# kemingy/rabitq

Hardware: AMD Instinct MI355X
Metric: queries/sec at recall@10>=0.95, 100Mx128; HBM GB/s on popcount scan (higher is better)
Workload: dtype exact integer dot (fp6 MFMA, v_dot8_u32_u4) + f32

## Files before the change

rabitq_amd/csrc/host_query.h:

```cpp
#pragma once
struct QueryParams {
    uint32_t nq, len, probe, topk;
    bool heuristic;
    uint32_t cap, hcap;
    const float *thr_init = nullptr;
    bool seg_final = false;
    bool ext_lists = false;
};

#define RQ_DEFAULT_CAP 4096u
#define RQ_MAX_CAP_HINT 32768u
#define RQ_MAX_NQ_PER_PASS 65536u
#define RQ_MAX_PROBE 16384u

static rq_status ws_prepare(const rq_index *idx, Workspace &ws, const QueryParams &qp) {
    const uint32_t nprobe = std::min(qp.probe, idx->k);
    const uint64_t nq = qp.nq, npairs = nq * nprobe;
    if (!ws.stream) HIPC(hipStreamCreateWithFlags(&ws.stream, hipStreamNonBlocking));
    if (!ws.h_totals) HIPC(hipHostMalloc((void **)&ws.h_totals, 16 * sizeof(unsigned long long)));
    RQC(ws.qpad.ensure(nq * idx->dim));
    RQC(ws.y.ensure(nq * idx->dim));
    if (!qp.ext_lists) RQC(ws.dist.ensure(nq * idx->k));
    RQC(ws.probe_dist.ensure(npairs));
    RQC(ws.probe_cluster.ensure(npairs));
// ... 418 lines not shown
        a.dbg = (uint32_t)g_scan_dbg.load();
        const uint32_t stage_tile = use_mfma ? scan_mfma_tile(W, arena_stage, additive) : tile;
        a.tiles_per_group = ceil_div(std::min<uint64_t>(idx->max_list_len, sg.s_hi), stage_tile);
        sp.tile_table = nullptr;
        const uint64_t grid_blocks = (uint64_t)k * a.tiles_per_group, real_tiles = idx->n / stage_tile + k;
        const int tt_opt = g_scan_tile_table.load();
        if (cluster_major && scan_is_fused(W) && sg.s_hi >= idx->max_list_len &&
            (tt_opt == 2 || (tt_opt == 1 && grid_blocks > 4 * real_tiles))) {
            uint32_t count = 0;
            sp.tile_table = get_tile_table(idx, stage_tile, &count);
            if (sp.tile_table) a.use_table = 1u, a.ngroups = count, a.tiles_per_group = 1u;
        }
        uint32_t dense_cells = 0;
        if (rq_large_batch(nq) && !use_mfma && scan_is_fused(W) && g_dense_dir.load() && sg.s_hi != 0xFFFFFFFFu &&
            !(qp.seg_final && span > qp.cap)) {
            const uint64_t cells = (uint64_t)((sg.s_hi - 1) >> 6) - (sg.s_lo >> 6) + 2ull * slot_hi + 2;
            if (cells <= qp.cap) dense_cells = (uint32_t)cells;
        }
        a.dense_dir = dense_cells ? 1u : 0u;
        QSeg seg = useg;
        bool runs_in_tmp = false;
        if (arena_stage) {
            uint64_t want = std::max<uint64_t>(idx->arena_hint.load(), (uint64_t)nq * qp.cap / 2);
            unsigned long long total_slots = 0;
            uint32_t arena_rsub = 0;
            bool arena_retried = false;
            ws.arena_failed = true;
#ifdef RQ_DEV_ABLATIONS
            if (g_seg_opt.load() == 3) {
                DevBuf<SurvRec> never;
                RQC(never.alloc(1ull << 46));
                return fail(RQ_ERR_OOM, "survivor arena: injected failure (developer hook survivor_segments = 3)");
            }
#endif
            for (int attempt = 0;; ++attempt) {
                want = std::min<uint64_t>(want, 0xFFFF0000ull);
                RQC(ws.arena_recs.ensure(want));
                RQC(ws.arena_runs.ensure(want));
                RQC(ws.arena_cur.ensure(RQ_ARENA_SHARDS + 4));
                RQC(ws.arena_fail.ensure(RQ_ARENA_SHARDS));
                HIPC(hipMemsetAsync(ws.arena_cur.p, 0, (RQ_ARENA_SHARDS + 4) * 8, st));
                HIPC(hipMemsetAsync(ws.arena_fail.p, 0xFF, RQ_ARENA_SHARDS * 4, st));
                ScanExtra hx{};
                RQC(ws.arena_places.ensure(want));
                hx.arena_places = ws.arena_places.p, hx.reserved = nullptr;
                hx.arena_recs = ws.arena_recs.p, hx.arena_runs = reinterpret_cast<uint4 *>(ws.arena_runs.p), hx.arena_cur = ws.arena_cur.p;
                hx.arena_fail = ws.arena_fail.p;
                {
                    const uint64_t have = std::min<uint64_t>(ws.arena_recs.count, ws.arena_runs.count);
                    hx.arena_sub = hx.arena_rsub = (uint32_t)(have * 7 / 8 / RQ_ARENA_SHARDS);
                    hx.arena_common = (uint32_t)std::min<uint64_t>(have - (uint64_t)hx.arena_sub * RQ_ARENA_SHARDS, 0xFFFFFF00ull);
                }
                arena_rsub = hx.arena_rsub;
                RQC(ws.scan_extra.ensure(1));
                HIPC(hipMemcpyAsync(ws.scan_extra.p, &hx, sizeof hx, hipMemcpyHostToDevice, st));
                a.x = ws.scan_extra.p;
                a.dense_dir = 0u;
                pf.begin(use_mfma ? PF_SCAN_MATRIX : PF_SCAN);
                if (use_mfma) launch_scan_mfma(sp, a, W, st, additive);
                else launch_scan(sp, a, W, st);
                pf.end();
                pf.begin(PF_GROUP);
                seg_exact_kernel<<<ceil_div(nq, 256), 256, 0, st>>>(ws.surv_cnt.p, nq, 64u, ws.q_cap.p);
                seg_scan_kernel<<<1, 1024, 0, st>>>(ws.q_cap.p, nq, ws.q_base.p, ws.arena_cur.p + RQ_ARENA_SHARDS + 1);
                unsigned long long tail[2] = {0, 0};
                HIPC(hipMemcpyAsync(tail, ws.arena_cur.p + RQ_ARENA_SHARDS, 16, hipMemcpyDeviceToHost, st));
                HIPC(hipStreamSynchronize(st));
                total_slots = tail[1];
                if (!(uint32_t)tail[0]) break;
                pf.end();
                if (attempt >= 6 || want >= 0xFFFF0000ull) return fail(RQ_ERR_OOM, "survivor arena kept overflowing");
                const uint64_t nblocks = a.use_table ? a.ngroups : (uint64_t)a.ngroups * a.tiles_per_group;
                HIPC(hipMemsetAsync(ws.surv_cnt.p, 0, (size_t)nq * sizeof(unsigned long long), st));
                want = std::max<uint64_t>(want * 2, 1u << 20);
                if (nblocks < RQ_ARENA_SHARDS) want = std::max<uint64_t>(want, 8 * total_slots + (1u << 16)), arena_retried = true;
                else want = std::max<uint64_t>(want, total_slots + total_slots / 4);
            }
            ws.arena_failed = false;
            {
                uint64_t cur = idx->arena_hint.load();
                const uint64_t learnt = std::max<uint64_t>(total_slots + total_slots * 3 / 5, arena_retried ? std::min<uint64_t>(want, 0xFFFF0000ull) : 0ull);
                while (cur < learnt && !const_cast<rq_index *>(idx)->arena_hint.compare_exchange_weak(cur, learnt)) {}
            }
            if (total_slots > ws.surv.count || total_slots > ws.runs.count || total_slots > ws.runs_tmp.count) {
                const uint64_t grow = total_slots + total_slots / 8;
                RQC(ws.surv.ensure(grow));
                RQC(ws.runs.ensure(grow));
                RQC(ws.runs_tmp.ensure(grow));
            }
            sp.surv = ws.surv.p, sp.runs = ws.runs.p;
            arena_scatter_kernel<<<dim3(RQ_ARENA_SHARDS + RQ_ARENA_COMMON_BLOCKS, 2), 256, 0, st>>>(ws.arena_recs.p, reinterpret_cast<const uint4 *>(ws.arena_runs.p), ws.arena_cur.p,
                                                                              ws.arena_fail.p, arena_rsub, ws.q_base.p, ws.arena_places.p, ws.surv.p, ws.runs_tmp.p);
            runs_in_tmp = true;
            pf.end();
            seg = QSeg{ws.q_base.p, ws.q_cap.p, qp.cap};
            ws.pend_seg_slots = std::max<uint64_t>(ws.pend_seg_slots, total_slots);
        }
        if (dense_cells) {
            pf.begin(PF_SORT);
            clear_dir_kernel<<<ceil_div((uint64_t)nq * dense_cells, 256), 256, 0, st>>>(ws.runs.p, nq, seg, dense_cells);
            pf.end();
        }
        if (!arena_stage) {
            pf.begin(use_mfma ? PF_SCAN_MATRIX : PF_SCAN);
            if (use_mfma) launch_scan_mfma(sp, a, W, st, additive);
            else launch_scan(sp, a, W, st);
            pf.end();
        }
        if (use_mfma) ws.pend_matrix_stages++;
        if (prof_acc && additive) prof_acc->matrix_additive_launches++;
        if (prof_acc) prof_acc->scan_launches++;
        if (prof_acc && use_mfma) {
            prof_acc->matrix_launches++;
            ws.pend_matrix_ranges.push_back({sg.s_lo, sg.s_hi});
        }
        if (!rq_large_batch(nq) && qp.cap <= 4 * RQ_DEFAULT_CAP) {
            pf.begin(PF_RERANK);
            const uint32_t fin_threads = nq <= 16 ? 1024u : 256u;
            const uint32_t presorted = qp.cap > RQ_DEFAULT_CAP && nprobe <= 1024 ? 1u : 0u;
            if (presorted) {
                sort_runs_kernel<<<nq, 64, 0, st>>>(ws.runs.p, ws.surv_cnt.p, seg, ws.big_list.p, ws.big_list.p + nq, RQ_SORT_LDS_RECS, nullptr);
                sort_runs_mid_kernel<<<std::min(nq, 256u), 256, RQ_SORT_MID_LDS_WORDS * 8, st>>>(ws.runs.p, ws.use_runs_tmp ? ws.runs_tmp.p : nullptr, ws.surv_cnt.p,
                                                                                              seg, ws.big_list.p, ws.big_list.p + nq, nprobe, 0u,
                                                                                              RQ_SORT_MID_LDS_WORDS);
            }
            if (sb_fused_finish) {
                uint32_t flags = presorted;
                if (nq <= 32) {
                    accurate_kernel<<<dim3(std::max(1u, std::min(16u, 256u / nq)), nq), 256, (size_t)dim * sizeof(float), st>>>(
                        ws.surv.p, ws.surv_cnt.p, seg, idx->view(), qpad, dim, nullptr, probe_cluster, nprobe);
                    flags |= 2u;
                }
                const uint32_t presorted = flags;
                if (topk < 64)
                    sb_finish_kernel<true><<<nq, fin_threads, (size_t)dim * sizeof(float) + (2 * RQ_SBF_RUNS + RQ_SBF_RECS) * 16, st>>>(
                        ws.surv.p, ws.runs.p, ws.surv_cnt.p, seg, idx->view(), qpad, dim, topk, rs, probe_cluster, nprobe, presorted,
                        idx->map_ids.p, d_out_dist, d_out_id, d_out_n, ws.rough_cnt.p, ws.totals.p);
                else
                    sb_finish_kernel<false><<<nq, fin_threads, (size_t)dim * sizeof(float) + (2 * RQ_SBF_RUNS + RQ_SBF_RECS) * 16, st>>>(
                        ws.surv.p, ws.runs.p, ws.surv_cnt.p, seg, idx->view(), qpad, dim, topk, rs, probe_cluster, nprobe, presorted,
                        idx->map_ids.p, d_out_dist, d_out_id, d_out_n, ws.rough_cnt.p, ws.totals.p);
                sb_results_done = true;
            } else if (qp.heuristic)
                stage_finish_kernel<true><<<nq, fin_threads, (size_t)dim * sizeof(float), st>>>(ws.surv.p, ws.runs.p, ws.surv_cnt.p, seg, idx->view(),
                                                              qpad, dim, topk, rs, probe_cluster, nprobe, presorted);
            else
                stage_finish_kernel<false><<<nq, fin_threads, (size_t)dim * sizeof(float), st>>>(ws.surv.p, ws.runs.p, ws.surv_cnt.p, seg, idx->view(),
                                                               qpad, dim, topk, rs, probe_cluster, nprobe, presorted);
            pf.end();
        } else {
            pf.begin(PF_RERANK);
            const uint32_t gx = std::max(1u, std::min(16u, 4096u / std::max(nq, 1u)));
            if (idx->base_q8.p && (stage_no > 0 || qp.thr_init) && !(g_scan_dbg & 512))
                accurate_filtered8_kernel<<<dim3(gx, nq), 256, (size_t)dim * sizeof(float) + (nprobe <= RQ_ACC8_LDS_PROBES ? (size_t)nprobe * 16 : 0), st>>>(
                    ws.surv.p, ws.surv_cnt.p, seg, idx->base.p, idx->base_q8.p, idx->list_q8.p, qpad, dim, rerank_order, ws.thr.p,
                    probe_cluster, nprobe, ws.nshadow.p, k);
            else if (idx->base_h.p && (stage_no > 0 || qp.thr_init) && !(g_scan_dbg & 512))
                accurate_filtered_kernel<<<dim3(gx, nq), 256, (size_t)dim * sizeof(float), st>>>(
                    ws.surv.p, ws.surv_cnt.p, seg, idx->base.p, idx->base_h.p, qpad, dim, rerank_order, ws.thr.p,
                    ws.nshadow.p);
            else if (idx->split_rows && (stage_no > 0 || qp.thr_init) && !(g_scan_dbg & 512))
                accurate_split_kernel<<<dim3(gx, nq), 256, (size_t)dim * sizeof(float) + (nprobe <= RQ_ACC8_LDS_PROBES ? (size_t)nprobe * 16 : 0), st>>>(
                    ws.surv.p, ws.surv_cnt.p, seg, idx->view(), qpad, dim, rerank_order, ws.thr.p, probe_cluster, nprobe, ws.nshadow.p);
            else
                accurate_kernel<<<dim3(gx, nq), 256, (size_t)dim * sizeof(float), st>>>(ws.surv.p, ws.surv_cnt.p, seg, idx->view(), qpad, dim,
                                                                                        rerank_order, probe_cluster, nprobe);
            pf.end();
            if (!dense_cells) {
                pf.begin(PF_SORT);
                sort_runs_kernel<<<nq, 64, 0, st>>>(ws.runs.p, ws.surv_cnt.p, seg, ws.big_list.p, ws.big_list.p + nq, 512u,
                                                    runs_in_tmp ? ws.runs_tmp.p : nullptr);
                sort_runs_mid_kernel<<<mid_blocks, 256, RQ_SORT_MID_LDS_WORDS * 8, st>>>(ws.runs.p, (ws.use_runs_tmp || runs_in_tmp) ? ws.runs_tmp.p : nullptr,
                                                                                      ws.surv_cnt.p, seg, ws.big_list.p, ws.big_list.p + nq, nprobe,
                                                                                      runs_in_tmp ? 1u : 0u, RQ_SORT_MID_LDS_WORDS);
                pf.end();
            }
            pf.begin(PF_REPLAY);
            if (qp.heuristic)
                replay_kernel<true><<<nq, 64, 16, st>>>(ws.surv.p, ws.runs.p, ws.surv_cnt.p, seg, topk, rs, dense_cells);
            else if (topk < 64)
                replay_kernel<false, true><<<nq, 64, 16, st>>>(ws.surv.p, ws.runs.p, ws.surv_cnt.p, seg, topk, rs, dense_cells);
            else
                replay_kernel<false><<<nq, 64, (size_t)topk * 8, st>>>(ws.surv.p, ws.runs.p, ws.surv_cnt.p, seg, topk, rs, dense_cells);
            pf.end();
        }
    }

    pf.begin(PF_REPLAY);
    if (sb_results_done) {
    } else {
    if (qp.heuristic) {
        sort_survivors_kernel<<<nq, 256, 0, st>>>(ws.arr.p, ws.arr_len.p, qp.hcap);
        finalize_heuristic_kernel<<<ceil_div((uint64_t)nq * topk, 256), 256, 0, st>>>(rs, nq, topk, d_row_map, idx->map_ids.p,
                                                                                       d_out_dist, d_out_id, d_out_n);
    } else {
        finalize_heap_kernel<<<ceil_div((uint64_t)nq * topk, 256), 256, 0, st>>>(rs, nq, topk, d_row_map, idx->map_ids.p, d_out_dist,
                                                                                  d_out_id, d_out_n);
    }
    metrics_sum_kernel<<<std::min(256u, ceil_div(nq, 256)), 256, 0, st>>>(
        ws.rough_cnt.p, ws.precise.p, ws.need.p, qp.heuristic ? ws.arr_len.p : nullptr, ws.nsurv.p, ws.nshadow.p, nq, ws.ovf.p, qp.hcap,
        ws.totals.p);
    }
    pf.end();
    if (pf.on) (void)hipEventRecord(pf.spans[total_span].b, st);
    HIPC(hipMemcpyAsync(ws.h_totals, ws.totals.p, 7 * sizeof(unsigned long long), hipMemcpyDeviceToHost, st));
    ws.h_totals[7] = 0, ws.h_totals[8] = 0, ws.h_totals[9] = 0, ws.h_totals[10] = 0;
    if (ws.pend_prefiltered) HIPC(hipMemcpyAsync(ws.h_totals + 10, ws.totals.p + 12, 8, hipMemcpyDeviceToHost, st));
    if (ws.pend_matrix_stages) {
        stat_fold_kernel<<<1, 64, 0, st>>>(ws.stat.p, ws.stat.p + 200);
        HIPC(hipMemcpyAsync(ws.h_totals + 8, ws.stat.p + 200, 16, hipMemcpyDeviceToHost, st));
    }
    if (rq_large_batch(nq))
        HIPC(hipMemcpyAsync(ws.h_totals + 7, ws.big_list.p + nq + 2, 4, hipMemcpyDeviceToHost, st));
    ws.pend_total_span = total_span;
    ws.pend_nq = nq;
    ws.pend_cap = qp.cap;
    if (defer) return RQ_OK;
    return finish_pass(idx, ws, res, prof_acc);
}

static Workspace *ws_acquire(rq_index *idx) {
    std::lock_guard<std::mutex> g(idx->ws_mu);
    for (auto &w : idx->ws_pool)
        if (!w->busy) {
            w->busy = true;
            return w.get();
        }
    idx->ws_pool.emplace_back(new Workspace());
    idx->ws_pool.back()->busy = true;
    return idx->ws_pool.back().get();
}
static void ws_release(rq_index *idx, Workspace *w) {
    std::lock_guard<std::mutex> g(idx->ws_mu);
    w->busy = false;
}

static rq_status validate_query(const rq_index *idx, const float *d_q, uint32_t len, uint32_t probe, uint32_t topk,
                                const float *d_out_dist, const uint32_t *d_out_id, const uint32_t *d_out_n) {
    RQC(ensure_device());
    RQC(ensure_kernel_attributes());
    if (!idx || !d_q || !d_out_dist || !d_out_id || !d_out_n) return fail(RQ_ERR_INVALID, "null argument");
    if (idx->dim != (len + 63) / 64 * 64)
        return fail(RQ_ERR_DIM_MISMATCH, "query length " + std::to_string(len) + " does not pad to index dim " +
                                             std::to_string(idx->dim));
    if (probe == 0 || idx->k == 0) return fail(RQ_ERR_INVALID, "probe == 0 (the reference panics at rabitq.rs:295)");
    if (topk == 0 || topk > RQ_MAX_TOPK) return fail(RQ_ERR_UNSUPPORTED, "topk must be in [1, 2048]");
    if (std::min(probe, idx->k) > RQ_MAX_PROBE) return fail(RQ_ERR_UNSUPPORTED, "probe > 16384 not supported");
    if (idx->dim > 4096) return fail(RQ_ERR_UNSUPPORTED, "dim > 4096 not supported");
    return RQ_OK;
}

static uint32_t pass_capacity(const rq_index *idx, uint32_t remaining, bool seeded, bool *seg) {
    const uint32_t hint = idx->cap_hint.load();
    const int opt = g_seg_opt.load();
    *seg = !seeded && rq_large_batch(remaining) && scan_is_fused(idx->W) && (opt >= 2 || (opt == 1 && hint > RQ_DEFAULT_CAP));
    if (*seg) return RQ_DEFAULT_CAP;
    return std::max(RQ_DEFAULT_CAP, hint);
}

static uint32_t pass_queries(const rq_index *idx, uint32_t remaining, uint32_t probe, uint32_t cap0, bool seg, bool ext_lists = false) {
    const uint64_t slot_bytes = cap0 > RQ_DEFAULT_CAP || seg || idx->big_dirs_hint.load() > 0 ? 48 : 32;
    const uint64_t max_nq = ext_lists ? 16ull * RQ_MAX_NQ_PER_PASS : RQ_MAX_NQ_PER_PASS, max_pairs = ext_lists ? (1ull << 26) : (1ull << 22);
    uint32_t step_nq = (uint32_t)std::min<uint64_t>(std::min<uint64_t>(remaining, max_nq),
                                                    std::max<uint64_t>(1, idx->pass_budget / ((uint64_t)cap0 * slot_bytes)));
    return std::min<uint32_t>(step_nq, (uint32_t)std::max<uint64_t>(1, max_pairs / std::min(probe, idx->k)));
}

static rq_status after_pass(rq_index *idx, Workspace *ws, const QueryParams &qp, const float *d_q, float *d_out_dist,
                            uint32_t *d_out_id, uint32_t *d_out_n, const uint32_t *ext_cluster, const float *ext_dist,
                            const PassResult &pr, rq_profile_t &prof, uint64_t &tot_precise) {
    const uint32_t len = qp.len, probe = qp.probe, topk = qp.topk;
    const bool heuristic = qp.heuristic;
    const uint32_t npb = std::min(probe, idx->k);
    if (pr.max_need > qp.cap) {
        uint32_t want = pow2_ceil((uint32_t)std::min<uint64_t>(pr.max_need + pr.max_need / 4, RQ_MAX_CAP_HINT));
        uint32_t cur = idx->cap_hint.load();
        while (cur < want && !idx->cap_hint.compare_exchange_weak(cur, want)) {}
    }
    if (!pr.overflowed) return RQ_OK;
    uint32_t cap = qp.cap, hcap = qp.hcap;
    std::vector<uint32_t> h_need(qp.nq), h_alen(qp.nq), h_ovf(qp.nq), over_rows;
    HIPC(hipMemcpy(h_need.data(), ws->need.p, qp.nq * 4, hipMemcpyDeviceToHost));
    HIPC(hipMemcpy(h_alen.data(), ws->arr_len.p, qp.nq * 4, hipMemcpyDeviceToHost));
    HIPC(hipMemcpy(h_ovf.data(), ws->ovf.p, qp.nq * 4, hipMemcpyDeviceToHost));
    uint32_t max_need = 0, max_alen = 0;
    for (uint32_t b = 0; b < qp.nq; ++b)
        if (h_ovf[b] || (heuristic && h_alen[b] > hcap)) {
            over_rows.push_back(b);
            max_need = std::max(max_need, h_need[b]);
            max_alen = std::max(max_alen, h_alen[b]);
        }
    int guard = 0;
    while (!over_rows.empty() && guard++ < 8) {
        prof.retries += (uint32_t)over_rows.size();
        uint32_t ncap = std::max(cap * 2, pow2_ceil(max_need));
        uint32_t nhcap = heuristic ? std::max(hcap * 2, pow2_ceil(std::max(max_alen, max_need))) : hcap;
        uint32_t chunk = (uint32_t)std::max<uint64_t>(1, (4ull << 30) / ((uint64_t)(ncap + nhcap) * sizeof(SurvRec)));
        std::vector<uint32_t> still;
        Workspace *rwsp = ws_acquire(idx);
        struct RelR {
            rq_index *i;
            Workspace *w;
            ~RelR() { ws_release(i, w); }
        } relr{idx, rwsp};
        Workspace &rws = *rwsp;
        DevBuf<float> &sub_q = rws.retry_q;
        DevBuf<uint32_t> &sub_rows = rws.retry_rows;
// ... 281 lines not shown
```

rabitq_amd/csrc/kernels_query.h:

```cpp
#pragma once
#ifndef RQ_COLLECT_UNROLL
#define RQ_COLLECT_UNROLL 8
#endif
#include "common.h"
#include "kernels_scan_common.h"

#pragma clang fp contract(off)

__global__ void pad_rows_kernel(const float *__restrict__ in, float *__restrict__ out, uint64_t n,
                                uint32_t len, uint32_t dim) {
    uint64_t i = (uint64_t)blockIdx.x * blockDim.x + threadIdx.x;
    if (i >= n * dim) return;
    uint64_t r = i / dim;
    uint32_t c = (uint32_t)(i - r * dim);
    out[i] = c < len ? in[r * len + c] : 0.0f;
}

__global__ __launch_bounds__(256) void rotate_valu_kernel(const float *__restrict__ x,
                                                          const float *__restrict__ P,
                                                          float *__restrict__ out, uint64_t n,
                                                          uint32_t dim) {
    uint64_t r = (uint64_t)blockIdx.x * 4 + threadIdx.y;
    uint32_t j = blockIdx.y * 64 + threadIdx.x;
    if (r >= n) return;
    const float *xr = x + r * dim;
    float acc[8] = {0, 0, 0, 0, 0, 0, 0, 0};
    for (uint32_t c = 0; c < dim; c += 8) {
#pragma unroll
        for (int l = 0; l < 8; ++l) acc[l] = fmaf(xr[c + l], P[(uint64_t)(c + l) * dim + j], acc[l]);
    }
    out[r * dim + j] = reduce8_regs(acc);
}

template <int QT>
__global__ __launch_bounds__(256) void coarse_dist_sreg_kernel(const float *__restrict__ cent_t,
                                                               const float *__restrict__ y, float *__restrict__ dist,
                                                               uint32_t k, uint32_t dim, uint32_t nq, uint32_t kstride) {
    const uint32_t q0 = blockIdx.x * QT;
    const uint32_t j = blockIdx.y * 256 + threadIdx.x;
    const bool live = j < k;
    const float *cp = cent_t + (live ? j : 0);
    f32x2 acc[QT][4];
#pragma unroll
    for (int v = 0; v < QT; ++v)
#pragma unroll
        for (int l = 0; l < 4; ++l) acc[v][l] = f32x2{0.0f, 0.0f};
    static_assert(QT % 4 == 0, "queries are fetched four at a time");
    for (uint32_t c = 0; c < dim; c += 16) {
        float ce[16];
#pragma unroll
        for (int l = 0; l < 16; ++l) ce[l] = cp[(uint64_t)(c + l) * kstride];
#pragma unroll
        for (int v0 = 0; v0 < QT; v0 += 4) {
            float yv[4][16];
#pragma unroll
            for (int v = 0; v < 4; ++v) {
                const uint32_t q = q0 + v0 + v < nq ? q0 + v0 + v : nq - 1;
                const float *yq = y + (uint64_t)q * dim + c;
#pragma unroll
                for (int l = 0; l < 16; ++l) yv[v][l] = yq[l];
            }
#pragma unroll
            for (int h = 0; h < 2; ++h)
#pragma unroll
                for (int v = 0; v < 4; ++v)
#pragma unroll
                    for (int l = 0; l < 4; ++l) {
                        const f32x2 c2 = {ce[8 * h + 2 * l], ce[8 * h + 2 * l + 1]};
                        const f32x2 y2 = {yv[v][8 * h + 2 * l], yv[v][8 * h + 2 * l + 1]};
                        const f32x2 d2 = c2 - y2;
                        acc[v0 + v][l] = __builtin_elementwise_fma(d2, d2, acc[v0 + v][l]);
                    }
        }
    }
    if (live) {
#pragma unroll
        for (int v = 0; v < QT; ++v) {
            float a[8];
#pragma unroll
            for (int l = 0; l < 4; ++l) a[2 * l] = acc[v][l].x, a[2 * l + 1] = acc[v][l].y;
            if (q0 + v < nq) dist[(uint64_t)(q0 + v) * k + j] = reduce8_regs(a);
        }
    }
}

template <int QT>
__global__ __launch_bounds__(256) void coarse_dist_kernel(const float *__restrict__ cent_t,
                                                          const float *__restrict__ y,
                                                          float *__restrict__ dist, uint32_t k,
                                                          uint32_t dim, uint32_t nq, uint32_t kstride) {
    extern __shared__ __attribute__((aligned(16))) float ys[];
    const uint32_t q0 = blockIdx.x * QT;
    const uint32_t j = blockIdx.y * 256 + threadIdx.x;
    for (uint32_t i = threadIdx.x; i < QT * dim; i += 256) {
        uint32_t v = i / dim, e = i - v * dim;
        ys[e * QT + v] = (q0 + v < nq) ? y[(uint64_t)(q0 + v) * dim + e] : 0.0f;
    }
    __syncthreads();
    static_assert(QT % 4 == 0, "queries are processed in packed pairs, read four at a time");
    f32x2 acc[QT / 2][8];
#pragma unroll
    for (int v = 0; v < QT / 2; ++v)
#pragma unroll
        for (int l = 0; l < 8; ++l) acc[v][l] = f32x2{0.0f, 0.0f};
    const bool live = j < k;
    const float *cp = cent_t + (live ? j : 0);
    for (uint32_t c = 0; c < dim; c += 8) {
        float ce[8];
#pragma unroll
        for (int l = 0; l < 8; ++l) ce[l] = cp[(uint64_t)(c + l) * kstride];
#pragma unroll
        for (int l = 0; l < 8; ++l) {
            const f32x2 ce2 = {ce[l], ce[l]};
#pragma unroll
            for (int v4 = 0; v4 < QT / 4; ++v4) {
                const float4 yq = *reinterpret_cast<const float4 *>(&ys[(c + l) * QT + 4 * v4]);
                const f32x2 y01 = {yq.x, yq.y}, y23 = {yq.z, yq.w};
                const f32x2 d01 = ce2 - y01, d23 = ce2 - y23;
                acc[2 * v4][l] = __builtin_elementwise_fma(d01, d01, acc[2 * v4][l]);
                acc[2 * v4 + 1][l] = __builtin_elementwise_fma(d23, d23, acc[2 * v4 + 1][l]);
            }
        }
    }
    if (live) {
#pragma unroll
        for (int v = 0; v < QT / 2; ++v) {
            float a0[8], a1[8];
#pragma unroll
            for (int l = 0; l < 8; ++l) a0[l] = acc[v][l].x, a1[l] = acc[v][l].y;
            if (q0 + 2 * v < nq) dist[(uint64_t)(q0 + 2 * v) * k + j] = reduce8_regs(a0);
            if (q0 + 2 * v + 1 < nq) dist[(uint64_t)(q0 + 2 * v + 1) * k + j] = reduce8_regs(a1);
        }
    }
}

template <typename T, typename KeyFn>
__device__ __forceinline__ void bitonic_sort_block(T *a, uint32_t n, KeyFn key) {
    if (n < 2) return;
    uint32_t p2 = 1;
    while (p2 < n) p2 <<= 1;
    const uint32_t half = p2 >> 1;
    for (uint32_t k = 2; k <= p2; k <<= 1) {
        for (uint32_t t = threadIdx.x; t < half; t += blockDim.x) {
            uint32_t hk = k >> 1;
            uint32_t blk = t / hk, off = t - blk * hk;
            uint32_t i = blk * k + off, j = blk * k + k - 1 - off;
            if (j < n) {
                T ai = a[i], aj = a[j];
                if (key(aj) < key(ai)) {
                    a[i] = aj;
                    a[j] = ai;
                }
            }
        }
        __syncthreads();
        for (uint32_t s = k >> 2; s >= 1; s >>= 1) {
            for (uint32_t t = threadIdx.x; t < half; t += blockDim.x) {
                uint32_t i = (t / s) * (2 * s) + (t % s), j = i + s;
// ... 2023 lines not shown
            if (!rr.split) ++rejected;
#endif
            if (rr.split) {
                const uint16_t *x = reinterpret_cast<const uint16_t *>(rr.p) + 8 * hf;
                float d0 = 0.0f, d1 = 0.0f, n0 = 0.0f, n1 = 0.0f;
                for (uint32_t c = 0; c < dim; c += 128) {
                    uint4 xv[8];
                    const bool full = dim - c >= 128;
#pragma unroll
                    for (int u = 0; u < 8; ++u)
                        if (u < 4 || full) xv[u] = *reinterpret_cast<const uint4 *>(x + c + 16 * u);
#pragma unroll
                    for (int u = 0; u < 8; ++u) {
                        if (!(u < 4 || full)) continue;
                        const float4 qa = *reinterpret_cast<const float4 *>(acc_q + c + 16 * u + 8 * hf);
                        const float4 qb = *reinterpret_cast<const float4 *>(acc_q + c + 16 * u + 8 * hf + 4);
                        const float x0 = __builtin_bit_cast(float, xv[u].x << 16), x1 = __builtin_bit_cast(float, xv[u].x & 0xFFFF0000u);
                        const float x2 = __builtin_bit_cast(float, xv[u].y << 16), x3 = __builtin_bit_cast(float, xv[u].y & 0xFFFF0000u);
                        const float x4 = __builtin_bit_cast(float, xv[u].z << 16), x5 = __builtin_bit_cast(float, xv[u].z & 0xFFFF0000u);
                        const float x6 = __builtin_bit_cast(float, xv[u].w << 16), x7 = __builtin_bit_cast(float, xv[u].w & 0xFFFF0000u);
                        const float e0 = x0 - qa.x, e1 = x1 - qa.y, e2 = x2 - qa.z, e3 = x3 - qa.w;
                        const float e4 = x4 - qb.x, e5 = x5 - qb.y, e6 = x6 - qb.z, e7 = x7 - qb.w;
                        d0 = fmaf(e0, e0, d0), d1 = fmaf(e1, e1, d1), d0 = fmaf(e2, e2, d0), d1 = fmaf(e3, e3, d1);
                        d0 = fmaf(e4, e4, d0), d1 = fmaf(e5, e5, d1), d0 = fmaf(e6, e6, d0), d1 = fmaf(e7, e7, d1);
                        n0 = fmaf(x0, x0, n0), n1 = fmaf(x1, x1, n1), n0 = fmaf(x2, x2, n0), n1 = fmaf(x3, x3, n1);
                        n0 = fmaf(x4, x4, n0), n1 = fmaf(x5, x5, n1), n0 = fmaf(x6, x6, n0), n1 = fmaf(x7, x7, n1);
                    }
                }
                float dt = d0 + d1, nx = n0 + n1;
                dt += __shfl_xor(dt, 1, 2), nx += __shfl_xor(nx, 1, 2);
                const float err = (sqrtf(nx) * up) * 3.9216e-3f + 1.0e-37f;
                const float t = sqrtf(dt * down) * down - err * up;
                if (t > 0.0f && (t * t) * (down * down) > thr) {
                    exact = false;
                    if (hf == 0) recs[i].accurate = __builtin_inff();
#ifndef RQ_EXP_COUNT_HOST
                    ++rejected;
#endif
                }
            }
        }
        if (exact && hf == 0) queue[atomicAdd(&qn, 1u)] = i;
        __syncthreads();
        const uint32_t waiting = qn;
        __syncthreads();
        if (waiting >= 128) {
            exact_of(queue[waiting - 128 + pair]);
            if (threadIdx.x == 0) qn = waiting - 128;
            __syncthreads();
        }
    }
    const uint32_t waiting = qn;
    if (pair < waiting) exact_of(queue[pair]);
    uint32_t rj = hf == 0 ? rejected : 0u;
#pragma unroll
    for (int o = 32; o >= 1; o >>= 1) rj += __shfl_xor(rj, o, 64);
    if ((threadIdx.x & 63) == 0 && rj) atomicAdd(&nshadow[b], rj);
}

__host__ __device__ __forceinline__ bool q8_row_norms(uint32_t dim) {
    const uint32_t tpr = dim / 16;
    return tpr >= 1 && tpr <= 64 && (tpr & (tpr - 1)) == 0;
}
__global__ __launch_bounds__(256) void q8_range_kernel(const float *__restrict__ base, const uint32_t *__restrict__ offsets, uint32_t dim,
                                                       float4 *__restrict__ list_q8) {
    __shared__ float smn[4], smx[4];
    __shared__ uint32_t sbad[4];
    const uint32_t c = blockIdx.x;
    const uint64_t e0 = (uint64_t)offsets[c] * dim, e1 = (uint64_t)offsets[c + 1] * dim;
    float mn = 3.402823466e+38f, mx = -3.402823466e+38f;
    uint32_t bad = 0;
    for (uint64_t e = e0 + threadIdx.x * 4ull; e < e1; e += 1024) {
        const float4 v = *reinterpret_cast<const float4 *>(base + e);
        const float ve[4] = {v.x, v.y, v.z, v.w};
#pragma unroll
        for (int i = 0; i < 4; ++i) {
            if (!(fabsf(ve[i]) < 3.0e38f)) bad = 1;
            mn = ve[i] < mn ? ve[i] : mn;
            mx = ve[i] > mx ? ve[i] : mx;
        }
    }
#pragma unroll
    for (int o = 32; o >= 1; o >>= 1) {
        const float a = __shfl_xor(mn, o, 64), b = __shfl_xor(mx, o, 64);
        mn = a < mn ? a : mn, mx = b > mx ? b : mx;
        bad |= __shfl_xor(bad, o, 64);
    }
    if ((threadIdx.x & 63) == 0) smn[threadIdx.x >> 6] = mn, smx[threadIdx.x >> 6] = mx, sbad[threadIdx.x >> 6] = bad;
    __syncthreads();
    if (threadIdx.x == 0) {
        for (int w = 1; w < 4; ++w) mn = smn[w] < mn ? smn[w] : mn, mx = smx[w] > mx ? smx[w] : mx, bad |= sbad[w];
        float lo = mn, sc = (mx - mn) * (1.0f / 255.0f);
        if (e1 == e0) lo = 0.0f, sc = 1.0f;
        if (!(sc > 0.0f)) sc = 1.0f;
        if (!(sc < 3.0e38f) || !(fabsf(lo) < 3.0e38f)) bad = 1;
        list_q8[c] = make_float4(bad ? 0.0f : lo, bad ? 1.0f : sc, bad ? __builtin_inff() : 0.0f, bad ? __builtin_inff() : 0.0f);
    }
}
__global__ __launch_bounds__(256) void q8_encode_kernel(const float *__restrict__ base, const uint32_t *__restrict__ offsets, uint32_t dim,
                                                        float4 *__restrict__ list_q8, uint8_t *__restrict__ out) {
    __shared__ float smax[4], snorm[4];
    const uint32_t c = blockIdx.y, r0 = offsets[c] + blockIdx.x * 256u, r1 = offsets[c + 1];
    if (r0 >= r1) return;
    const float4 par = list_q8[c];
    const float lo = par.x, sc = par.y, inv = 1.0f / sc;
    const uint32_t tpr = dim / 16, rows_per_pass = 256 / tpr;
    const uint32_t rr = threadIdx.x / tpr, g = threadIdx.x - rr * tpr;
    const bool row_norms = q8_row_norms(dim);
    float emax = 0.0f, nmax = 0.0f;
    for (uint32_t r = r0 + rr; r < r1 && r < r0 + 256u && rr < rows_per_pass; r += rows_per_pass) {
        float e2 = 0.0f;
        const float *x = base + (uint64_t)r * dim + 16 * g;
        uint32_t w[4];
#pragma unroll
        for (int u = 0; u < 4; ++u) {
            const float4 v = *reinterpret_cast<const float4 *>(x + 4 * u);
            const float ve[4] = {v.x, v.y, v.z, v.w};
            w[u] = 0;
#pragma unroll
            for (int i = 0; i < 4; ++i) {
                float t = rintf((ve[i] - lo) * inv);
                t = t < 0.0f ? 0.0f : (t > 255.0f ? 255.0f : t);
                const uint32_t code = (uint32_t)t;
                const float e = fabsf(ve[i] - fmaf(sc, (float)code, lo));
                emax = (e > emax || !(e < 3.0e38f)) ? (e < 3.0e38f ? e : __builtin_inff()) : emax;
                e2 = fmaf(e, e, e2);
                w[u] |= code << (8 * i);
            }
        }
        *reinterpret_cast<uint4 *>(out + (uint64_t)r * dim + 16 * g) = make_uint4(w[0], w[1], w[2], w[3]);
        if (row_norms) {
            for (uint32_t o = tpr >> 1; o >= 1; o >>= 1) e2 += __shfl_xor(e2, (int)o, 64);
            nmax = (e2 > nmax || !(e2 < 3.0e38f)) ? (e2 < 3.0e38f ? e2 : __builtin_inff()) : nmax;
        }
    }
#pragma unroll
    for (int o = 32; o >= 1; o >>= 1) {
        const float a = __shfl_xor(emax, o, 64), b = __shfl_xor(nmax, o, 64);
        emax = a > emax ? a : emax, nmax = b > nmax ? b : nmax;
    }
    if ((threadIdx.x & 63) == 0) smax[threadIdx.x >> 6] = emax, snorm[threadIdx.x >> 6] = nmax;
    __syncthreads();
    if (threadIdx.x == 0) {
        for (int w2 = 1; w2 < 4; ++w2) emax = smax[w2] > emax ? smax[w2] : emax, nmax = snorm[w2] > nmax ? snorm[w2] : nmax;
        atomicMax(reinterpret_cast<unsigned int *>(&list_q8[c].z), __builtin_bit_cast(unsigned int, emax));
        const float nrm = sqrtf(nmax) * (1.0f + (float)(dim + 8) * 6.0e-8f);
        if (row_norms) atomicMax(reinterpret_cast<unsigned int *>(&list_q8[c].w), __builtin_bit_cast(unsigned int, nrm));
    }
}

#ifndef RQ_ACC8_WAVES
#define RQ_ACC8_WAVES 4
#endif
__global__ __launch_bounds__(256, RQ_ACC8_WAVES) void accurate_filtered8_kernel(SurvRec *__restrict__ surv,
                                                                 const unsigned long long *__restrict__ surv_cnt,
                                                                 const QSeg seg, const float *__restrict__ base,
                                                                 const uint8_t *__restrict__ base_q8, const float4 *__restrict__ list_q8,
                                                                 const float *__restrict__ qpad, uint32_t dim,
                                                                 const uint32_t *__restrict__ order,
                                                                 const float *__restrict__ thr_start,
                                                                 const uint32_t *__restrict__ probe_cluster, uint32_t nprobe,
                                                                 uint32_t *__restrict__ nshadow, uint32_t nlists) {
    extern __shared__ __attribute__((aligned(16))) float acc_q[];
    __shared__ uint32_t queue[512];
    __shared__ uint32_t qn;
    const uint32_t b = order ? order[blockIdx.y] : blockIdx.y;
    const uint32_t n = (uint32_t)surv_cnt[b];
    if (n > seg.capof(b) || n == 0) return;
    SurvRec *recs = surv + seg.at(b);
    const uint32_t hf = threadIdx.x & 1, pair = threadIdx.x >> 1;
    const uint32_t i_first = blockIdx.x * 256;
    SurvRec nxt[2];
    nxt[0] = recs[i_first + pair < n ? i_first + pair : 0u], nxt[1] = recs[i_first + 128 + pair < n ? i_first + 128 + pair : 0u];
    const uint32_t *pc = probe_cluster + (uint64_t)b * nprobe;
    float4 *lpar = reinterpret_cast<float4 *>(acc_q + dim);
    const bool par_lds = nprobe <= RQ_ACC8_LDS_PROBES;
    for (uint32_t c = threadIdx.x * 4; c < dim; c += 1024)
        *reinterpret_cast<float4 *>(acc_q + c) = *reinterpret_cast<const float4 *>(qpad + (uint64_t)b * dim + c);
    if (par_lds)
        for (uint32_t sl = threadIdx.x; sl < nprobe; sl += 256)
            lpar[sl] = pc[sl] < nlists ? list_q8[pc[sl]] : make_float4(0.0f, 1.0f, __builtin_inff(), __builtin_inff());
    if (threadIdx.x == 0) qn = 0;
    __syncthreads();
    const float thr = thr_start[b];
    const bool test = thr > 1e-30f && thr < 3.0e38f;
    const float eps = (float)(dim / 4 + 64) * 5.9604645e-8f, down = 1.0f - eps, up = 1.0f + eps;
    const float sqd = sqrtf((float)dim) * 1.001f;
    const bool rown = q8_row_norms(dim);
    const uint32_t ngrp = dim / 16;
    uint32_t rejected = 0;
    for (uint32_t i0 = i_first; i0 < n; i0 += gridDim.x * 256) {
        uint32_t iv[2] = {i0 + pair, i0 + 128 + pair};
        bool exact[2] = {iv[0] < n, iv[1] < n};
        const SurvRec cur[2] = {nxt[0], nxt[1]};
        {
            const uint32_t j0 = i0 + gridDim.x * 256 + pair, j1 = j0 + 128;
            nxt[0] = recs[j0 < n ? j0 : 0u], nxt[1] = recs[j1 < n ? j1 : 0u];
        }
        if (test) {
            float4 par[2];
            const uint8_t *x[2];
#pragma unroll
            for (int v = 0; v < 2; ++v) {
                par[v] = par_lds ? lpar[cur[v].slot] : list_q8[pc[cur[v].slot]];
                x[v] = base_q8 + (uint64_t)cur[v].pos * dim;
            }
            float d0[2] = {0.0f, 0.0f}, d1[2] = {0.0f, 0.0f};
            for (uint32_t g0 = hf; g0 < ngrp; g0 += 8) {
                uint4 cv[2][4];
#pragma unroll
                for (int v = 0; v < 2; ++v)
#pragma unroll
                    for (int u = 0; u < 4; ++u)
                        if (g0 + 2 * u < ngrp) cv[v][u] = *reinterpret_cast<const uint4 *>(x[v] + 16 * (g0 + 2 * u));
#pragma unroll
                for (int u = 0; u < 4; ++u) {
                    if (!(g0 + 2 * u < ngrp)) continue;
                    const float *q = acc_q + 16 * (g0 + 2 * u);
#pragma unroll
                    for (int wi = 0; wi < 4; ++wi) {
                        const float4 qa = *reinterpret_cast<const float4 *>(q + 4 * wi);
#pragma unroll
                        for (int v = 0; v < 2; ++v) {
                            const uint32_t wv = wi == 0 ? cv[v][u].x : (wi == 1 ? cv[v][u].y : (wi == 2 ? cv[v][u].z : cv[v][u].w));
                            const float e0 = fmaf(par[v].y, (float)(wv & 255u), par[v].x) - qa.x;
                            const float e1 = fmaf(par[v].y, (float)((wv >> 8) & 255u), par[v].x) - qa.y;
                            const float e2 = fmaf(par[v].y, (float)((wv >> 16) & 255u), par[v].x) - qa.z;
                            const float e3 = fmaf(par[v].y, (float)(wv >> 24), par[v].x) - qa.w;
                            d0[v] = fmaf(e0, e0, d0[v]), d1[v] = fmaf(e1, e1, d1[v]), d0[v] = fmaf(e2, e2, d0[v]), d1[v] = fmaf(e3, e3, d1[v]);
                        }
                    }
                    asm volatile("" ::: "memory");
                }
            }
#pragma unroll
            for (int v = 0; v < 2; ++v) {
                float dt = d0[v] + d1[v];
                dt += __shfl_xor(dt, 1, 2);
                const float err = rown ? par[v].w * up : (par[v].z * up) * sqd;
                const float t = sqrtf(dt * down) * down - err * up;
                if (exact[v] && t > 0.0f && (t * t) * (down * down) > thr) {
                    exact[v] = false;
                    if (hf == 0) recs[iv[v]].accurate = __builtin_inff();
                    ++rejected;
                }
            }
        }
#pragma unroll
        for (int v = 0; v < 2; ++v)
            if (exact[v] && hf == 0) queue[atomicAdd(&qn, 1u)] = iv[v];
        __syncthreads();
        uint32_t waiting = qn;
        __syncthreads();
        while (waiting >= 128) {
            const uint32_t j = queue[waiting - 128 + pair];
            const float r = exact_l2_pair(base + (uint64_t)recs[j].pos * dim + 4 * hf, acc_q, dim, hf);
            if (hf == 0) recs[j].accurate = r;
            waiting -= 128;
            __syncthreads();
            if (threadIdx.x == 0) qn = waiting;
            __syncthreads();
        }
    }
    const uint32_t waiting = qn;
    if (pair < waiting) {
        const uint32_t j = queue[pair];
        const float r = exact_l2_pair(base + (uint64_t)recs[j].pos * dim + 4 * hf, acc_q, dim, hf);
        if (hf == 0) recs[j].accurate = r;
    }
    uint32_t rj = hf == 0 ? rejected : 0u;
#pragma unroll
    for (int o = 32; o >= 1; o >>= 1) rj += __shfl_xor(rj, o, 64);
    if ((threadIdx.x & 63) == 0 && rj) atomicAdd(&nshadow[b], rj);
}

__global__ __launch_bounds__(256) void accurate_kernel(SurvRec *__restrict__ surv,
                                                       const unsigned long long *__restrict__ surv_cnt,
                                                       const QSeg seg, const BaseView base,
                                                       const float *__restrict__ qpad, uint32_t dim,
                                                       const uint32_t *__restrict__ order,
                                                       const uint32_t *__restrict__ probe_cluster, uint32_t nprobe) {
    extern __shared__ __attribute__((aligned(16))) float acc_q[];
    const uint32_t b = order ? order[blockIdx.y] : blockIdx.y;
    const uint32_t n = (uint32_t)surv_cnt[b];
    if (n > seg.capof(b) || n == 0) return;
    for (uint32_t c = threadIdx.x * 4; c < dim; c += 1024)
        *reinterpret_cast<float4 *>(acc_q + c) = *reinterpret_cast<const float4 *>(qpad + (uint64_t)b * dim + c);
    __syncthreads();
    accurate_rows(surv + seg.at(b), n, base, acc_q, dim, blockIdx.x * 128 + (threadIdx.x >> 1), gridDim.x * 128,
                  probe_cluster + (uint64_t)b * nprobe);
}

__global__ __launch_bounds__(64) void sort_runs_kernel(RunRec *__restrict__ runs,
                                                        const unsigned long long *__restrict__ surv_cnt,
                                                        const QSeg seg, uint32_t *__restrict__ big_list,
                                                        uint32_t *__restrict__ big_count, uint32_t list_above,
                                                        const RunRec *runs_src) {
    const uint32_t b = blockIdx.x;
    const unsigned long long c = surv_cnt[b];
    if ((uint32_t)c > seg.capof(b)) return;
    const uint32_t nruns = (uint32_t)(c >> 32);
    if (list_above != 512u) {
        if (nruns > list_above && threadIdx.x == 0) big_list[atomicAdd(big_count, 1u)] = b;
        return;
    }
    if (nruns > 512) {
        if (threadIdx.x == 0) big_list[atomicAdd(big_count, 1u)] = b;
        return;
    }
    sort_segment<RunRec, 512>(runs + seg.at(b), nruns, runs_src ? runs_src + seg.at(b) : nullptr);
}

__global__ __launch_bounds__(256) void sort_runs_mid_kernel(RunRec *__restrict__ runs, RunRec *__restrict__ runs_tmp,
                                                            const unsigned long long *__restrict__ surv_cnt, const QSeg seg,
                                                            const uint32_t *__restrict__ big_list,
                                                            uint32_t *__restrict__ big_count ,
                                                            uint32_t nslots, uint32_t src_is_tmp, uint32_t lds_words) {
    extern __shared__ __attribute__((aligned(16))) uint32_t mid_lds[];
    const uint32_t total = big_count[0];
    for (uint32_t i = blockIdx.x; i < total; i += gridDim.x) {
        const uint32_t b = big_list[i], n = (uint32_t)(surv_cnt[b] >> 32);
        RunRec *dir = runs + seg.at(b), *tmp = runs_tmp ? runs_tmp + seg.at(b) : nullptr;
        bool done = false;
        if (nslots <= 1024 && tmp && lds_words) {
            if (src_is_tmp) {
                done = order_runs_bitmap<1024>(tmp, dir, n, nslots, mid_lds, mid_lds + lds_words, lds_words);
            } else {
                done = order_runs_bitmap<1024>(dir, tmp, n, nslots, mid_lds, mid_lds + lds_words, lds_words);
                if (done) {
                    __threadfence_block();
                    __syncthreads();
                    for (uint32_t e = threadIdx.x; e < n; e += blockDim.x) dir[e] = tmp[e];
                }
            }
        }
        if (!done) {
            if (src_is_tmp && tmp) {
                __syncthreads();
                for (uint32_t e = threadIdx.x; e < n; e += blockDim.x) dir[e] = tmp[e];
                __threadfence_block();
                __syncthreads();
            }
            if (nslots <= 1024 && tmp) sort_runs_by_slot<1024>(dir, tmp, n, nslots);
            else sort_segment<RunRec, 16>(dir, n);
        }
        __syncthreads();
    }
    __syncthreads();
    if (threadIdx.x == 0) {
        __threadfence();
        if (atomicAdd(big_count + 1, 1u) + 1 == gridDim.x) {
            if (total > big_count[2]) big_count[2] = total;
            big_count[0] = 0;
            big_count[1] = 0;
        }
    }
}

template <bool HEURISTIC, bool REGHEAP = false>
__global__ __launch_bounds__(64) void replay_kernel(const SurvRec *__restrict__ surv, const RunRec *__restrict__ runs,
                                                    unsigned long long *__restrict__ surv_cnt, const QSeg seg, uint32_t topk,
                                                    ReplayState st, uint32_t dense_cells) {
    extern __shared__ __attribute__((aligned(16))) unsigned char replay_smem[];
    int32_t *hkey = reinterpret_cast<int32_t *>(replay_smem);
    uint32_t *hid = reinterpret_cast<uint32_t *>(replay_smem) + topk;
    const uint32_t b = blockIdx.x;
    const unsigned long long cnt64 = surv_cnt[b];
    const uint32_t cnt = (uint32_t)cnt64;
    const bool overflow = cnt > seg.capof(b);
    const uint32_t n = overflow ? 0 : cnt;
    const uint32_t nruns = overflow ? 0 : (dense_cells ? dense_cells : (uint32_t)(cnt64 >> 32));
    if (threadIdx.x == 0) {
        if (cnt > st.need[b]) st.need[b] = cnt;
        if (overflow) st.ovf[b] = 1u;
        st.nsurv[b] += n;
        surv_cnt[b] = 0;
    }
    if (n == 0) return;
    replay_wave<HEURISTIC, REGHEAP>(surv + seg.at(b), runs + seg.at(b), nruns, topk, b, st, hkey, hid);
}

__global__ void seg_exact_kernel(unsigned long long *__restrict__ surv_cnt, uint32_t nq, uint32_t floor_cap,
                                 uint32_t *__restrict__ q_cap) {
    const uint32_t b = blockIdx.x * blockDim.x + threadIdx.x;
    if (b >= nq) return;
    const uint32_t cnt = (uint32_t)surv_cnt[b];
    const uint32_t cap = cnt > floor_cap ? cnt : floor_cap;
    q_cap[b] = cap > 0xFFFFFF80u ? 0xFFFFFFC0u : ((cap + 63u) & ~63u);
}
__global__ __launch_bounds__(256) void arena_scatter_kernel(const SurvRec *__restrict__ arena_recs, const uint4 *__restrict__ arena_runs,
                                                            const unsigned long long *__restrict__ arena_cur,
                                                            const unsigned int *__restrict__ arena_fail, uint32_t arena_rsub,
                                                            const unsigned long long *__restrict__ q_base,
                                                            const uint2 *__restrict__ arena_places, SurvRec *__restrict__ surv,
                                                            RunRec *__restrict__ runs) {
    __shared__ uint32_t s_pref[4][65], s_src[4][64];
    __shared__ unsigned long long s_dst[4][64];
    const bool common = blockIdx.x >= RQ_ARENA_SHARDS;
    const uint32_t shard = common ? RQ_ARENA_SHARDS : blockIdx.x;
    uint32_t nr;
    if (!common) {
        nr = (uint32_t)(arena_cur[shard] >> 32);
// ... 191 lines not shown
```

Baseline: 3.854 million.

## Replace float shadow-distance filter with integer udot4 expansion and per-slot bounds

The q8 prefilter in the accurate rerank kernel no longer decodes each 8-bit code to float and accumulates squared error. The query is quantized to 16-bit codes split into high and low byte planes in LDS, and v_dot4 integer dot products accumulate q·x, x·x and sum(x). The squared distance is then reconstructed in double with a rigorous error bound. Per-list rejection limits are precomputed into LDS slots, and rows per thread become a macro (default 2). This trades VALU float work for integer dots plus some double-precision epilogue math and extra LDS, and it risks overflow or bound subtleties.

Result: no change. 3.899 million, median of 6 (+1.2%).

```diff
diff --git a/rabitq_amd/csrc/host_query.h b/rabitq_amd/csrc/host_query.h
--- a/rabitq_amd/csrc/host_query.h
+++ b/rabitq_amd/csrc/host_query.h
@@ -594,7 +594,7 @@
             pf.begin(PF_RERANK);
             const uint32_t gx = std::max(1u, std::min(16u, 4096u / std::max(nq, 1u)));
             if (idx->base_q8.p && (stage_no > 0 || qp.thr_init) && !(g_scan_dbg & 512))
-                accurate_filtered8_kernel<<<dim3(gx, nq), 256, (size_t)dim * sizeof(float) + (nprobe <= RQ_ACC8_LDS_PROBES ? (size_t)nprobe * 16 : 0), st>>>(
+                accurate_filtered8_kernel<<<dim3(gx, nq), 256, (size_t)dim * (sizeof(float) + 2) + (nprobe <= RQ_ACC8_LDS_PROBES ? (size_t)nprobe * sizeof(Q8Slot) : 0), st>>>(
                     ws.surv.p, ws.surv_cnt.p, seg, idx->base.p, idx->base_q8.p, idx->list_q8.p, qpad, dim, rerank_order, ws.thr.p,
                     probe_cluster, nprobe, ws.nshadow.p, k);
             else if (idx->base_h.p && (stage_no > 0 || qp.thr_init) && !(g_scan_dbg & 512))
diff --git a/rabitq_amd/csrc/kernels_query.h b/rabitq_amd/csrc/kernels_query.h
--- a/rabitq_amd/csrc/kernels_query.h
+++ b/rabitq_amd/csrc/kernels_query.h
@@ -4,6 +4,7 @@
 #endif
 #include "common.h"
 #include "kernels_scan_common.h"
+#include "q8_bound.h"
 
 #pragma clang fp contract(off)
 
@@ -2333,6 +2334,18 @@
 #ifndef RQ_ACC8_WAVES
 #define RQ_ACC8_WAVES 4
 #endif
+#ifndef RQ_ACC8_ROWS
+#define RQ_ACC8_ROWS 2
+#endif
+struct Q8Slot {
+    float lo, s;
+    double R;
+};
+__device__ __forceinline__ double rq_uniform_f64(double v) {
+    const uint64_t u = __builtin_bit_cast(uint64_t, v);
+    const uint32_t lo = __builtin_amdgcn_readfirstlane((uint32_t)u), hi = __builtin_amdgcn_readfirstlane((uint32_t)(u >> 32));
+    return __builtin_bit_cast(double, ((uint64_t)hi << 32) | lo);
+}
 __global__ __launch_bounds__(256, RQ_ACC8_WAVES) void accurate_filtered8_kernel(SurvRec *__restrict__ surv,
                                                                  const unsigned long long *__restrict__ surv_cnt,
                                                                  const QSeg seg, const float *__restrict__ base,
@@ -2343,84 +2356,132 @@
                                                                  const uint32_t *__restrict__ probe_cluster, uint32_t nprobe,
                                                                  uint32_t *__restrict__ nshadow, uint32_t nlists) {
     extern __shared__ __attribute__((aligned(16))) float acc_q[];
-    __shared__ uint32_t queue[512];
+    constexpr uint32_t NR = RQ_ACC8_ROWS, PER = 128 * NR;
+    __shared__ uint32_t queue[128 + PER];
     __shared__ uint32_t qn;
     const uint32_t b = order ? order[blockIdx.y] : blockIdx.y;
     const uint32_t n = (uint32_t)surv_cnt[b];
     if (n > seg.capof(b) || n == 0) return;
     SurvRec *recs = surv + seg.at(b);
-    const uint32_t hf = threadIdx.x & 1, pair = threadIdx.x >> 1;
-    const uint32_t i_first = blockIdx.x * 256;
-    SurvRec nxt[2];
-    nxt[0] = recs[i_first + pair < n ? i_first + pair : 0u], nxt[1] = recs[i_first + 128 + pair < n ? i_first + 128 + pair : 0u];
+    const uint32_t hf = threadIdx.x & 1, pair = threadIdx.x >> 1, lane = threadIdx.x & 63;
+    const uint32_t i_first = blockIdx.x * PER;
+    SurvRec nxt[NR];
+#pragma unroll
+    for (uint32_t v = 0; v < NR; ++v) nxt[v] = recs[i_first + 128 * v + pair < n ? i_first + 128 * v + pair : 0u];
     const uint32_t *pc = probe_cluster + (uint64_t)b * nprobe;
-    float4 *lpar = reinterpret_cast<float4 *>(acc_q + dim);
+    uint8_t *qh = reinterpret_cast<uint8_t *>(acc_q + dim), *ql = qh + dim;
+    Q8Slot *lpar = reinterpret_cast<Q8Slot *>(ql + dim);
     const bool par_lds = nprobe <= RQ_ACC8_LDS_PROBES;
     for (uint32_t c = threadIdx.x * 4; c < dim; c += 1024)
         *reinterpret_cast<float4 *>(acc_q + c) = *reinterpret_cast<const float4 *>(qpad + (uint64_t)b * dim + c);
+    float4 lraw[RQ_ACC8_LDS_PROBES / 256];
     if (par_lds)
-        for (uint32_t sl = threadIdx.x; sl < nprobe; sl += 256)
-            lpar[sl] = pc[sl] < nlists ? list_q8[pc[sl]] : make_float4(0.0f, 1.0f, __builtin_inff(), __builtin_inff());
+#pragma unroll
+        for (uint32_t k = 0; k < RQ_ACC8_LDS_PROBES / 256; ++k) {
+            const uint32_t sl = threadIdx.x + 256 * k;
+            if (sl < nprobe) lraw[k] = pc[sl] < nlists ? list_q8[pc[sl]] : make_float4(0.0f, 1.0f, __builtin_inff(), __builtin_inff());
+        }
     if (threadIdx.x == 0) qn = 0;
     __syncthreads();
     const float thr = thr_start[b];
-    const bool test = thr > 1e-30f && thr < 3.0e38f;
-    const float eps = (float)(dim / 4 + 64) * 5.9604645e-8f, down = 1.0f - eps, up = 1.0f + eps;
-    const float sqd = sqrtf((float)dim) * 1.001f;
+    bool test = thr > 1e-30f && thr < 3.0e38f;
+    float qmax = 0.0f;
+    uint32_t bad = 0;
+    for (uint32_t c = 4 * lane; c < dim; c += 256) {
+        const float4 v = *reinterpret_cast<const float4 *>(acc_q + c);
+        const float a = fabsf(v.x), a1 = fabsf(v.y), a2 = fabsf(v.z), a3 = fabsf(v.w);
+        if (!(((a + a1) + (a2 + a3)) < 3.0e38f)) bad = 1;
+        qmax = fmaxf(qmax, fmaxf(fmaxf(a, a1), fmaxf(a2, a3)));
+    }
+#pragma unroll
+    for (int o = 32; o >= 1; o >>= 1) qmax = fmaxf(qmax, __shfl_xor(qmax, o, 64)), bad |= __shfl_xor(bad, o, 64);
+    test = test && !bad;
+    Q8Query qc = {1.0, 0.0, 0.0, 0.0};
+    double T = 0.0;
+    if (test) {
+        const float sigma = q8_query_sigma(qmax);
+        int32_t sum_q = 0;
+        double sum_q2 = 0.0, sum_r2 = 0.0;
+        for (uint32_t c = 4 * lane; c < dim; c += 256) {
+            const float4 v = *reinterpret_cast<const float4 *>(acc_q + c);
+            const float e[4] = {v.x, v.y, v.z, v.w};
+            uint32_t wh = 0, wl = 0;
+#pragma unroll
+            for (int i = 0; i < 4; ++i) {
+                const int32_t Q = q8_query_code(e[i], sigma);
+                sum_q += Q, sum_q2 += (double)(Q * Q), sum_r2 += q8_query_resid2(e[i], sigma, Q);
+                const uint32_t u = (uint32_t)(Q + 32768);
+                wh |= (u >> 8) << (8 * i), wl |= (u & 255u) << (8 * i);
+            }
+            if (threadIdx.x < 64) reinterpret_cast<uint32_t *>(qh)[c / 4] = wh, reinterpret_cast<uint32_t *>(ql)[c / 4] = wl;
+        }
+#pragma unroll
+        for (int o = 32; o >= 1; o >>= 1)
+            sum_q += __shfl_xor(sum_q, o, 64), sum_q2 += __shfl_xor(sum_q2, o, 64), sum_r2 += __shfl_xor(sum_r2, o, 64);
+        qc = q8_query_consts(sigma, sum_q, sum_q2, sum_r2);
+        qc.sigma = rq_uniform_f64(qc.sigma), qc.sq = rq_uniform_f64(qc.sq), qc.qq = rq_uniform_f64(qc.qq), qc.rq = rq_uniform_f64(qc.rq);
+        T = rq_uniform_f64(q8_thr_root(thr, dim));
+    }
     const bool rown = q8_row_norms(dim);
+    auto slot_of = [&](const float4 &par) {
+        return Q8Slot{par.x, par.y, q8_slot_limit(par.x, par.y, q8_list_err(par.z, par.w, dim, rown), dim, qc.rq, T)};
+    };
+    if (par_lds && test)
+#pragma unroll
+        for (uint32_t k = 0; k < RQ_ACC8_LDS_PROBES / 256; ++k)
+            if (threadIdx.x + 256 * k < nprobe) lpar[threadIdx.x + 256 * k] = slot_of(lraw[k]);
+    __syncthreads();
     const uint32_t ngrp = dim / 16;
     uint32_t rejected = 0;
-    for (uint32_t i0 = i_first; i0 < n; i0 += gridDim.x * 256) {
-        uint32_t iv[2] = {i0 + pair, i0 + 128 + pair};
-        bool exact[2] = {iv[0] < n, iv[1] < n};
-        const SurvRec cur[2] = {nxt[0], nxt[1]};
-        {
-            const uint32_t j0 = i0 + gridDim.x * 256 + pair, j1 = j0 + 128;
-            nxt[0] = recs[j0 < n ? j0 : 0u], nxt[1] = recs[j1 < n ? j1 : 0u];
+    for (uint32_t i0 = i_first; i0 < n; i0 += gridDim.x * PER) {
+        uint32_t iv[NR];
+        bool exact[NR];
+        SurvRec cur[NR];
+#pragma unroll
+        for (uint32_t v = 0; v < NR; ++v) {
+            iv[v] = i0 + 128 * v + pair, exact[v] = iv[v] < n, cur[v] = nxt[v];
+            const uint32_t j = i0 + gridDim.x * PER + 128 * v + pair;
+            nxt[v] = recs[j < n ? j : 0u];
         }
         if (test) {
-            float4 par[2];
-            const uint8_t *x[2];
-#pragma unroll
-            for (int v = 0; v < 2; ++v) {
-                par[v] = par_lds ? lpar[cur[v].slot] : list_q8[pc[cur[v].slot]];
-                x[v] = base_q8 + (uint64_t)cur[v].pos * dim;
-            }
-            float d0[2] = {0.0f, 0.0f}, d1[2] = {0.0f, 0.0f};
+            const uint8_t *x[NR];
+#pragma unroll
+            for (uint32_t v = 0; v < NR; ++v) x[v] = base_q8 + (uint64_t)cur[v].pos * dim;
+            uint32_t ah[NR], al[NR], c2[NR], c1[NR];
+#pragma unroll
+            for (uint32_t v = 0; v < NR; ++v) ah[v] = al[v] = c2[v] = c1[v] = 0u;
             for (uint32_t g0 = hf; g0 < ngrp; g0 += 8) {
-                uint4 cv[2][4];
-#pragma unroll
-                for (int v = 0; v < 2; ++v)
+                uint4 cv[NR][4];
+#pragma unroll
+                for (uint32_t v = 0; v < NR; ++v)
 #pragma unroll
                     for (int u = 0; u < 4; ++u)
                         if (g0 + 2 * u < ngrp) cv[v][u] = *reinterpret_cast<const uint4 *>(x[v] + 16 * (g0 + 2 * u));
 #pragma unroll
                 for (int u = 0; u < 4; ++u) {
                     if (!(g0 + 2 * u < ngrp)) continue;
-                    const float *q = acc_q + 16 * (g0 + 2 * u);
-#pragma unroll
-                    for (int wi = 0; wi < 4; ++wi) {
-                        const float4 qa = *reinterpret_cast<const float4 *>(q + 4 * wi);
-#pragma unroll
-                        for (int v = 0; v < 2; ++v) {
-                            const uint32_t wv = wi == 0 ? cv[v][u].x : (wi == 1 ? cv[v][u].y : (wi == 2 ? cv[v][u].z : cv[v][u].w));
-                            const float e0 = fmaf(par[v].y, (float)(wv & 255u), par[v].x) - qa.x;
-                            const float e1 = fmaf(par[v].y, (float)((wv >> 8) & 255u), par[v].x) - qa.y;
-                            const float e2 = fmaf(par[v].y, (float)((wv >> 16) & 255u), par[v].x) - qa.z;
-                            const float e3 = fmaf(par[v].y, (float)(wv >> 24), par[v].x) - qa.w;
-                            d0[v] = fmaf(e0, e0, d0[v]), d1[v] = fmaf(e1, e1, d1[v]), d0[v] = fmaf(e2, e2, d0[v]), d1[v] = fmaf(e3, e3, d1[v]);
+                    const uint4 uh = *reinterpret_cast<const uint4 *>(qh + 16 * (g0 + 2 * u));
+                    const uint4 ul = *reinterpret_cast<const uint4 *>(ql + 16 * (g0 + 2 * u));
+#pragma unroll
+                    for (uint32_t v = 0; v < NR; ++v) {
+                        const uint32_t w[4] = {cv[v][u].x, cv[v][u].y, cv[v][u].z, cv[v][u].w};
+                        const uint32_t h[4] = {uh.x, uh.y, uh.z, uh.w}, l[4] = {ul.x, ul.y, ul.z, ul.w};
+#pragma unroll
+                        for (int wi = 0; wi < 4; ++wi) {
+                            ah[v] = __builtin_amdgcn_udot4(w[wi], h[wi], ah[v], false);
+                            al[v] = __builtin_amdgcn_udot4(w[wi], l[wi], al[v], false);
+                            c2[v] = __builtin_amdgcn_udot4(w[wi], w[wi], c2[v], false);
+                            c1[v] = __builtin_amdgcn_udot4(w[wi], 0x01010101u, c1[v], false);
                         }
                     }
-                    asm volatile("" ::: "memory");
                 }
             }
 #pragma unroll
-            for (int v = 0; v < 2; ++v) {
-                float dt = d0[v] + d1[v];
-                dt += __shfl_xor(dt, 1, 2);
-                const float err = rown ? par[v].w * up : (par[v].z * up) * sqd;
-                const float t = sqrtf(dt * down) * down - err * up;
-                if (exact[v] && t > 0.0f && (t * t) * (down * down) > thr) {
+            for (uint32_t v = 0; v < NR; ++v) {
+                ah[v] += __shfl_xor(ah[v], 1, 2), al[v] += __shfl_xor(al[v], 1, 2);
+                c2[v] += __shfl_xor(c2[v], 1, 2), c1[v] += __shfl_xor(c1[v], 1, 2);
+                const Q8Slot p = par_lds ? lpar[cur[v].slot] : slot_of(list_q8[pc[cur[v].slot]]);
+                if (exact[v] && q8_shadow_l2_lo(p.lo, p.s, dim, qc, ah[v], al[v], c2[v], c1[v]) > p.R) {
                     exact[v] = false;
                     if (hf == 0) recs[iv[v]].accurate = __builtin_inff();
                     ++rejected;
@@ -2428,7 +2489,7 @@
             }
         }
 #pragma unroll
-        for (int v = 0; v < 2; ++v)
+        for (uint32_t v = 0; v < NR; ++v)
             if (exact[v] && hf == 0) queue[atomicAdd(&qn, 1u)] = iv[v];
         __syncthreads();
         uint32_t waiting = qn;
diff --git a/rabitq_amd/csrc/q8_bound.h b/rabitq_amd/csrc/q8_bound.h
--- /dev/null
+++ b/rabitq_amd/csrc/q8_bound.h
@@ -0,0 +1,64 @@
+#pragma once
+#include <math.h>
+#include <stdint.h>
+
+#if defined(__HIPCC__) || defined(__HIP__)
+#define RQ_Q8_HD __host__ __device__ __forceinline__
+#else
+#define RQ_Q8_HD inline
+#endif
+
+#define RQ_Q8_UP 1.0000000000009095
+
+RQ_Q8_HD float q8_query_sigma(float qmax) { return qmax >= 1.0e-30f ? qmax / 32767.0f : 1.0f; }
+RQ_Q8_HD int32_t q8_query_code(float q, float sigma) {
+    float t = rintf(q / sigma);
+    t = t < -32767.0f ? -32767.0f : (t > 32767.0f ? 32767.0f : t);
+    return (int32_t)t;
+}
+RQ_Q8_HD double q8_query_resid2(float q, float sigma, int32_t Q) {
+    const double r = (double)q - (double)sigma * (double)Q;
+    return r * r;
+}
+
+struct Q8Query {
+    double sigma, sq, qq;
+    double rq;
+};
+RQ_Q8_HD Q8Query q8_query_consts(float sigma, int64_t sum_q, double sum_q2, double sum_r2) {
+    Q8Query c;
+    c.sigma = (double)sigma;
+    c.sq = c.sigma * (double)sum_q;
+    c.qq = (c.sigma * c.sigma) * sum_q2;
+    c.rq = sqrt(sum_r2) * (1.0 + 0x1p-38);
+    return c;
+}
+RQ_Q8_HD float q8_list_err(float z, float w, uint32_t dim, bool row_norms) {
+    const float up = 1.0f + (float)(dim / 4 + 64) * 5.9604645e-8f;
+    return row_norms ? w * up : (z * up) * (sqrtf((float)dim) * 1.001f);
+}
+RQ_Q8_HD double q8_thr_root(float thr, uint32_t dim) {
+    const double down = 1.0 - (double)(dim / 4 + 64) * 0x1p-24;
+    return sqrt((double)thr / down) * RQ_Q8_UP;
+}
+RQ_Q8_HD double q8_slot_limit(float lo, float s, float err, uint32_t dim, double rq, double T) {
+    const double a = fabs((double)lo), b = fabs((double)lo + 255.0 * (double)s);
+    const double m = (a > b ? a : b) * RQ_Q8_UP;
+    const double half_ulp = sqrt((double)dim) * RQ_Q8_UP * (m * 0x1p-24 + 0x1p-150);
+    const double e = (((double)err + half_ulp) + rq) * RQ_Q8_UP;
+    const double et = (e + T) * RQ_Q8_UP;
+    return (et * et) * RQ_Q8_UP;
+}
+RQ_Q8_HD double q8_shadow_l2_lo(float lo, float s, uint32_t dim, const Q8Query &q, uint32_t ah, uint32_t al, uint32_t c2,
+                                uint32_t c1) {
+    const double cq = (256.0 * (double)ah + (double)al) - 32768.0 * (double)c1;
+    const double dl = (double)lo, ds = (double)s;
+    const double t0 = (double)dim * (dl * dl);
+    const double t1 = 2.0 * ((dl * ds) * (double)c1);
+    const double t2 = (ds * ds) * (double)c2;
+    const double t3 = dl * q.sq;
+    const double t4 = (ds * q.sigma) * cq;
+    const double d2 = ((t0 + t1) + t2) - 2.0 * (t3 + t4) + q.qq;
+    const double mag = ((t0 + fabs(t1)) + t2) + 2.0 * (fabs(t3) + fabs(t4)) + q.qq;
+    return d2 - mag * 0x1p-44;
+}
```
